# mederrata/spmf

Measured on AMD Instinct MI355X. Metric: elbo_steps_per_sec, higher is better.
Workload: dtype f32

## Files before the change

spmf_amd/csrc/row_pass.hip:

```cpp
#include <algorithm>

#include "common.h"
#include "kernels.h"

namespace spmf {

#ifndef ROW_MAX_BLOCKS
#define ROW_MAX_BLOCKS 4096
#endif
#ifndef ROW_DYN_NUM
#define ROW_DYN_NUM 1
#define ROW_DYN_DEN 8
#endif
static_assert(ROW_MAX_BLOCKS <= spmf::kDetMaxBlocks,
              "the deterministic mode's per-workgroup slots (common.h kDetMaxBlocks) are sized for at most that many row-pass workgroups");
#ifndef ROW_GRP
#define ROW_GRP 4
#endif
#ifndef ROW_WAVES_PER_SIMD
#define ROW_WAVES_PER_SIMD 1
#endif

namespace {

__device__ __forceinline__ float* lds_dyn() {
  extern __shared__ __attribute__((aligned(16))) float spmf_row_lds[];
  return spmf_row_lds;
}

template <int FMT>
struct EntryRow {
  __amdgpu_buffer_rsrc_t a, b;
};
template <int FMT>
__device__ __forceinline__ EntryRow<FMT> entry_row(const int32_t* __restrict__ col, const float* __restrict__ val,
                                                   const uint32_t* __restrict__ ent, int start, int n) {
  EntryRow<FMT> r;
  start = __builtin_amdgcn_readfirstlane(start);
  n = __builtin_amdgcn_readfirstlane(n);
  if (FMT == 1) {
    r.a = __builtin_amdgcn_make_buffer_rsrc(const_cast<uint32_t*>(ent + start), 0, n * 4, 0x00020000);
    r.b = r.a;
  } else {
    r.a = __builtin_amdgcn_make_buffer_rsrc(const_cast<int32_t*>(col + start), 0, n * 4, 0x00020000);
    r.b = __builtin_amdgcn_make_buffer_rsrc(const_cast<float*>(val + start), 0, n * 4, 0x00020000);
  }
  return r;
}
template <int FMT, bool NT>
__device__ __forceinline__ void load_entry(const EntryRow<FMT>& r, int i, int& ra, float& rb) {
  constexpr int AUX = NT ? 2 : 0;
  ra = (int)__builtin_amdgcn_raw_buffer_load_b32(r.a, i * 4, 0, AUX);
  rb = FMT == 1 ? 0.f : __uint_as_float(__builtin_amdgcn_raw_buffer_load_b32(r.b, i * 4, 0, AUX));
}
template <int FMT>
__device__ __forceinline__ void unpack_entry(int ra, float rb, bool ok, int& c, float& x) {
  if (FMT == 1) {
    const uint32_t w = ok ? (uint32_t)ra : kPadWord;
    c = (int)(w >> 16);
    x = (float)(w & 0xffffu);
  } else {
    c = ok ? ra : kPadRow;
    x = ok ? rb : 0.f;
  }
}

template <bool BASE>
__device__ __forceinline__ int bperm_i(int base_bytes, int imm_lanes, int v) {
  if constexpr (BASE) return __builtin_amdgcn_ds_bpermute(base_bytes + imm_lanes * 4, v);
  else return __shfl(v, (base_bytes >> 2) + imm_lanes);
}
template <bool BASE>
__device__ __forceinline__ float bperm_f(int base_bytes, int imm_lanes, float v) {
  return __int_as_float(bperm_i<BASE>(base_bytes, imm_lanes, __float_as_int(v)));
}

template <int KP, int LIK, bool LDSPHI = false>
struct RowCtx {
  static constexpr int LPN = KP / 4;
  static constexpr int NPI = 64 / LPN;
  static constexpr int GRP = LPN < ROW_GRP ? LPN : ROW_GRP;
  static constexpr bool BPI = LPN <= 8 && LIK != 1;
  GTable Ap, Vp;
  const float* phi;
  const uint8_t* ctype;
  int lane, sub, grp;
  int bp_grp, bp_row;

  template <int CNT>
  __device__ __forceinline__ void s1_group(int c, float x, int g0, float4& zacc) const {
    float4 a[CNT];
    float xv[CNT];
#pragma unroll
    for (int j = 0; j < CNT; ++j) {
      const int d = bperm_i<BPI>(bp_grp, (g0 + j) * NPI, c);
      xv[j] = bperm_f<BPI>(bp_grp, (g0 + j) * NPI, x);
      a[j] = gather4<LPN>(Ap, d, sub);
    }
#pragma unroll
    for (int j = 0; j < CNT; ++j) zacc = fma4(xv[j], a[j], zacc);
  }
  __device__ __forceinline__ void sweep1(int c, float x, int nchunk, float4& zacc) const {
#pragma unroll
    for (int g0 = 0; g0 < LPN; g0 += GRP) {
      if (g0 * NPI < nchunk) s1_group<GRP>(c, x, g0, zacc);
    }
  }

  template <int CNT>
  __device__ __forceinline__ void s2_issue(int c, int g0, float4 (&vv)[LPN]) const {
#pragma unroll
    for (int j = 0; j < CNT; ++j) {
      const int d = bperm_i<BPI>(bp_grp, (g0 + j) * NPI, c);
      vv[g0 + j] = gather4<LPN>(Vp, d, sub);
    }
  }
  template <int CNT>
  __device__ __forceinline__ void s2_dots(int g0, const float4& z, float4 (&vv)[LPN], float& rmine) const {
#pragma unroll
    for (int j = 0; j < CNT; ++j) {
      const float dot = group_sum<LPN>(dot4(z, vv[g0 + j]));
      if (sub == g0 + j) rmine = dot;
    }
#pragma unroll
    for (int j = CNT; j < GRP; ++j) vv[g0 + j] = make_float4(0.f, 0.f, 0.f, 0.f);
  }
  template <int CNT>
  __device__ __forceinline__ void s2_back(float cc, int g0, const float4 (&vv)[LPN],
                                          float4& gz) const {
#pragma unroll
    for (int j = 0; j < CNT; ++j) {
      const float cb = bperm_f<BPI>(bp_row, g0 + j, cc);
      gz = fma4(cb, vv[g0 + j], gz);
    }
  }

  __device__ __forceinline__ void s2_load(int c, int nchunk, float4 (&vv)[LPN]) const {
#pragma unroll
    for (int g0 = 0; g0 < LPN; g0 += GRP) {
      if (g0 * NPI < nchunk) {
#pragma unroll
        for (int j = 0; j < GRP; ++j) {
          const int d = bperm_i<BPI>(bp_grp, (g0 + j) * NPI, c);
          vv[g0 + j] = gather4<LPN>(Vp, d, sub);
        }
      } else {
#pragma unroll
        for (int j = 0; j < GRP; ++j) vv[g0 + j] = make_float4(0.f, 0.f, 0.f, 0.f);
      }
    }
  }
  __device__ __forceinline__ void sweep2_loaded(int c, float x, int nchunk, const float4& z, float4& gz, float& ll,
                                                double& nnf, const float4 (&vv)[LPN]) const {
    float rmine = 0.f;
#pragma unroll
    for (int g0 = 0; g0 < LPN; g0 += GRP) {
      if (g0 * NPI < nchunk) {
#pragma unroll
        for (int j = 0; j < GRP; ++j) {
          const float dot = group_sum<LPN>(dot4(z, vv[g0 + j]));
          if (sub == g0 + j) rmine = dot;
        }
      }
    }
    s2_cells(c, x, nchunk, rmine, vv, gz, ll, nnf);
  }

  template <class Hook>
  __device__ __forceinline__ void sweep2(int c, float x, int nchunk, const float4& z, float4& gz, float& ll,
                                         double& nnf, Hook&& behind_last) const {
    float4 vv[LPN];
    float rmine = 0.f;
#pragma unroll
    for (int g0 = 0; g0 < LPN; g0 += GRP) {
      const bool occ = g0 * NPI < nchunk;
      if (occ) s2_issue<GRP>(c, g0, vv);
      if (g0 + GRP >= LPN) behind_last();
      if (occ) s2_dots<GRP>(g0, z, vv, rmine);
      else s2_dots<0>(g0, z, vv, rmine);
    }
    s2_cells(c, x, nchunk, rmine, vv, gz, ll, nnf);
  }
  __device__ __forceinline__ void s2_cells(int c, float x, int nchunk, float rmine, const float4 (&vv)[LPN],
                                           float4& gz, float& ll, double& nnf) const {
    const int slot = sub * NPI + grp;
    const float xs = __shfl(x, slot);
    const int cs = __shfl(c, slot);
    float cc = 0.f;
    if (slot < nchunk && xs > 0.f) {
      if (LIK == 2 || LIK == 4 || (LIK == 3 && ctype[cs])) {
        float ey = 1.f;
        const float fy = LIK == 4 ? expm1_dec(fminf(rmine, kYSat), ey) : rmine;
        const float lg = fy + (LDSPHI ? lds_dyn()[cs] : phi[cs]);
        if (lg > -INFINITY && lg < INFINITY) {
          ll = fmaf(xs, lg, ll);
          cc = LIK == 4 ? xs * ey : xs;
        } else {
          nnf += 1.0;
        }
      } else {
        float ey = 1.f;
        const float fy = LIK == 1 ? expm1_dec(fminf(rmine, kYSat), ey) : rmine;
        const float r = fy + (LDSPHI ? lds_dyn()[cs] : phi[cs]);
        if (r > 0.f && r < INFINITY) {
          ll = fmaf(xs, logf(r), ll);
          cc = xs * ey * __builtin_amdgcn_rcpf(r);
        } else {
          nnf += 1.0;
          cc = ey;
        }
      }
    }
#pragma unroll
    for (int g0 = 0; g0 < LPN; g0 += GRP) {
      if (g0 * NPI < nchunk) s2_back<GRP>(cc, g0, vv, gz);
    }
  }
};

}

template <int KP, int LIK, int BT = 256, int PACKED = 0>
__global__ __launch_bounds__(BT, BT == 256 ? ROW_WAVES_PER_SIMD : 4) void row_pass_kernel(
    int64_t B, const int32_t* __restrict__ row_ptr, const int32_t* __restrict__ col,
    const float* __restrict__ val, const float* __restrict__ row_scale,
    const float* __restrict__ Ap, const float* __restrict__ Vp, const float* __restrict__ phi,
    const double* __restrict__ dprep, float* __restrict__ z, float* __restrict__ gzs,
    double* __restrict__ dacc, int mode, const float* __restrict__ gzd,
    const uint8_t* __restrict__ ctype, int Dcols, int64_t dacc_stride,
    const uint32_t* __restrict__ ent, double* __restrict__ det_slots, int64_t det_stride, int dyn_tail) {
  if (gridDim.y > 1) {
    const size_t sd = blockIdx.y;
    Ap += sd * (size_t)Dcols * KP;
    Vp += sd * (size_t)Dcols * KP;
    phi += sd * (size_t)Dcols;
    dprep += sd * (size_t)kPrepSeg * (KP + 1);
    z += sd * (size_t)B * KP;
    gzs += sd * (size_t)B * KP;
    dacc += sd * (size_t)dacc_stride;
  }
  const bool encode_only = mode == 1;
  constexpr int LPN = KP / 4;
  constexpr bool LDSPHI = BT != 256;
  if (LDSPHI && !encode_only) {
    float* pl = lds_dyn();
    for (int i = threadIdx.x; i < Dcols; i += BT) pl[i] = phi[i];
    __syncthreads();
  }
  RowCtx<KP, LIK, LDSPHI> cx;
  cx.Ap = gtable(Ap, Dcols, KP);
  cx.Vp = gtable(Vp, Dcols, KP);
  cx.phi = phi;
  cx.ctype = ctype;
  cx.lane = threadIdx.x & 63;
  cx.sub = cx.lane % LPN;
  cx.grp = cx.lane / LPN;
  cx.bp_grp = cx.grp * 4;
  cx.bp_row = cx.grp * LPN * 4;
  const int lane = cx.lane, sub = cx.sub, grp = cx.grp;
  const int wave = (int)blockIdx.x * (BT / 64) + __builtin_amdgcn_readfirstlane((int)(threadIdx.x >> 6));
  const int nwaves = (int)gridDim.x * (BT / 64);
  const int Bn = (int)B;

  float4 veta4 = make_float4(0.f, 0.f, 0.f, 0.f);
  if (!encode_only && (mode != 2 || LIK == 3 || !gzd))
    veta4 = make_float4((float)prep_sum(dprep, KP, sub * 4 + 0), (float)prep_sum(dprep, KP, sub * 4 + 1),
                        (float)prep_sum(dprep, KP, sub * 4 + 2), (float)prep_sum(dprep, KP, sub * 4 + 3));
  double ll_acc = 0.0, zsq_acc = 0.0, nnf_acc = 0.0;
  float4 zsum = make_float4(0.f, 0.f, 0.f, 0.f);

  int B_static = Bn;
  int dyn_lo = Bn, dyn_hi = Bn;
  unsigned int* dyn_ctr = nullptr;
  if (dyn_tail && !det_slots && !encode_only) {
    const int per_wave = Bn / nwaves;
    if (per_wave >= 8) {
      int fixed = per_wave - (per_wave * ROW_DYN_NUM) / ROW_DYN_DEN;
      if (fixed < 2) fixed = 2;
      B_static = fixed * nwaves;
      const int r = (int)(wave & (kDaccRep - 1));
      const int each = (Bn - B_static + kDaccRep - 1) / kDaccRep;
      dyn_lo = B_static + r * each;
      dyn_hi = dyn_lo + each < Bn ? dyn_lo + each : Bn;
      if (dyn_lo > Bn) dyn_lo = Bn;
      dyn_ctr = reinterpret_cast<unsigned int*>(dacc + (size_t)r * (kDaccHead + KP) + kDaccDynSlot);
    }
  }
  auto fixed_next = [&](int cur) -> int {
    if (cur >= Bn) return Bn;
    if (cur + nwaves < B_static) return cur + nwaves;
    return dyn_ctr ? -1 : Bn;
  };
  auto take_dynamic = [&]() -> int {
    unsigned int k = 0;
    if (lane == 0) k = atomicAdd(dyn_ctr, 1u);
    k = (unsigned int)__builtin_amdgcn_readfirstlane((int)k);
    const int row = dyn_lo + (int)k;
    return row < dyn_hi ? row : Bn;
  };

  const __amdgpu_buffer_rsrc_t dyn_rsrc = __builtin_amdgcn_make_buffer_rsrc(
      dyn_ctr ? dyn_ctr : reinterpret_cast<unsigned int*>(dacc), 0, dyn_ctr ? 4 : 0, 0x00020000);

  typedef const __attribute__((address_space(4))) int32_t* RowPtr;
  typedef const __attribute__((address_space(4))) float* RowScale;
  const RowPtr rptr = (RowPtr)row_ptr;
  const RowScale rscale = (RowScale)row_scale;
  int start = 0, end = 0, pc0 = 0, pc1 = 0, nstart = 0, nend = 0;
  float xi = 1.f, px0 = 0.f, px1 = 0.f, nxi = 1.f;
  int b = wave < B_static ? wave : Bn;
  int bn = fixed_next(b);
  if (bn < 0) bn = take_dynamic();
  int bnn = fixed_next(bn);
  if (bnn < 0) bnn = take_dynamic();
  if (b < Bn) {
    start = rptr[b];
    end = rptr[b + 1];
    xi = row_scale ? rscale[b] : 1.f;
    const EntryRow<PACKED> er = entry_row<PACKED>(col, val, ent, start, end - start);
    load_entry<PACKED, true>(er, lane, pc0, px0);
    load_entry<PACKED, true>(er, lane + 64, pc1, px1);
  }
  if (bn < Bn) {
    nstart = rptr[bn];
    nend = rptr[bn + 1];
    nxi = row_scale ? rscale[bn] : 1.f;
  }
  while (b < Bn) {
    const int n = end - start;
    int qc0 = 0, qc1 = 0, nnstart = 0, nnend = 0;
    float qx0 = 0.f, qx1 = 0.f, nnxi = 1.f;
    int bnnn = fixed_next(bnn);
    const bool dyn_ask = bnnn < 0;
    unsigned int dyn_k = 0;
    auto issue_next = [&]() {
      issue_fence(PACKED ? (const void*)ent : (const void*)col, val, row_ptr);
      dyn_k = (unsigned int)__builtin_amdgcn_raw_ptr_buffer_atomic_add_i32(1, dyn_rsrc, (dyn_ask && lane == 0) ? 0 : 4,
                                                                       0, 0);
      const EntryRow<PACKED> er = entry_row<PACKED>(col, val, ent, nstart, nend - nstart);
      load_entry<PACKED, true>(er, lane, qc0, qx0);
      load_entry<PACKED, true>(er, lane + 64, qc1, qx1);
      if (bnn < Bn) {
        nnstart = rptr[bnn];
        nnend = rptr[bnn + 1];
        nnxi = row_scale ? rscale[bnn] : 1.f;
      }
      issue_fence(PACKED ? (const void*)ent : (const void*)col, val, row_ptr);
    };
    constexpr bool BEHIND = KP <= 32;
    if constexpr (!BEHIND) issue_next();
    float4 zacc = make_float4(0.f, 0.f, 0.f, 0.f);
    float4 gz = make_float4(0.f, 0.f, 0.f, 0.f);
    float llrow = 0.f;
    if (n <= 128) {
      int c0, c1;
      float x0, x1;
      unpack_entry<PACKED>(pc0, px0, lane < n, c0, x0);
      unpack_entry<PACKED>(pc1, px1, lane + 64 < n, c1, x1);
      int n0 = min(n, 64);
      const int n1 = n - 64;
      if (mode != 2) {
        cx.sweep1(c0, x0, n0, zacc);
        if (n1 > 0) cx.sweep1(c1, x1, n1, zacc);
        zacc = across_groups_sum4<LPN>(zacc);
        zacc.x *= xi; zacc.y *= xi; zacc.z *= xi; zacc.w *= xi;
        if (grp == 0) reinterpret_cast<float4*>(z)[(size_t)b * LPN + sub] = zacc;
      } else {
        zacc = gather4<LPN>(z, (int)b, sub);
      }
      if (encode_only) {
        if constexpr (BEHIND) issue_next();
      } else {
        if constexpr (KP <= 32) {
          float4 vv[LPN];
          if (n1 > 0) {
            cx.s2_load(c0, n0, vv);
            cx.sweep2_loaded(c0, x0, n0, zacc, gz, llrow, nnf_acc, vv);
            c0 = c1; x0 = x1; n0 = n1;
          }
          cx.s2_load(c0, n0, vv);
          issue_next();
          cx.sweep2_loaded(c0, x0, n0, zacc, gz, llrow, nnf_acc, vv);
        } else {
          cx.sweep2(c0, x0, n0, zacc, gz, llrow, nnf_acc, [] {});
          if (n1 > 0) cx.sweep2(c1, x1, n1, zacc, gz, llrow, nnf_acc, [] {});
        }
      }
    } else {
      const EntryRow<PACKED> er = entry_row<PACKED>(col, val, ent, start, n);
      if (mode != 2) {
        int ra = pc0, ra1 = pc1;
        float rb = px0, rb1 = px1;
        for (int base = start; base < end; base += 64) {
          const int i2 = base + 128 + lane;
          int ra2;
          float rb2;
          load_entry<PACKED, false>(er, i2 - start, ra2, rb2);
          int c;
          float x;
          unpack_entry<PACKED>(ra, rb, base + lane < end, c, x);
          cx.sweep1(c, x, min(64, end - base), zacc);
          ra = ra1; rb = rb1; ra1 = ra2; rb1 = rb2;
        }
        zacc = across_groups_sum4<LPN>(zacc);
        zacc.x *= xi; zacc.y *= xi; zacc.z *= xi; zacc.w *= xi;
        if (grp == 0) reinterpret_cast<float4*>(z)[(size_t)b * LPN + sub] = zacc;
      } else {
        zacc = gather4<LPN>(z, (int)b, sub);
      }
      if (encode_only) {
        if constexpr (BEHIND) issue_next();
      } else {
        int ra = pc0, ra1 = pc1;
        float rb = px0, rb1 = px1;
        for (int base = start; base < end; base += 64) {
          const int i2 = base + 128 + lane;
          int ra2;
          float rb2;
          load_entry<PACKED, false>(er, i2 - start, ra2, rb2);
          int c;
          float x;
          unpack_entry<PACKED>(ra, rb, base + lane < end, c, x);
          if (BEHIND && base + 64 >= end) cx.sweep2(c, x, end - base, zacc, gz, llrow, nnf_acc, issue_next);
          else cx.sweep2(c, x, min(64, end - base), zacc, gz, llrow, nnf_acc, [] {});
          ra = ra1; rb = rb1; ra1 = ra2; rb1 = rb2;
        }
      }
    }
    const float xi_cur = xi;
    const int b_cur = b;
    start = nstart; end = nend; xi = nxi;
    pc0 = qc0; px0 = qx0; pc1 = qc1; px1 = qx1;
    nstart = nnstart; nend = nnend; nxi = nnxi;
    {
      const int row = dyn_lo + (int)(unsigned int)__builtin_amdgcn_readfirstlane((int)dyn_k);
      if (dyn_ask) bnnn = row < dyn_hi ? row : Bn;
    }
    b = bn; bn = bnn; bnn = bnnn;
    if (encode_only) continue;
    gz = across_groups_sum4<LPN>(gz);
    if (grp == 0) {
      zsq_acc += (double)dot4(zacc, zacc);
      zsum = add4(zsum, zacc);
      float4 dn = (mode == 2 && gzd) ? gather4<LPN>(gzd, (int)b_cur, sub) : veta4;
      if (LIK == 3 && mode == 2 && gzd) dn = add4(dn, veta4);
      if (mode == 3 && LIK != 3) dn = make_float4(0.f, 0.f, 0.f, 0.f);
      float4 o;
      o.x = xi_cur * (gz.x - dn.x - zacc.x);
      o.y = xi_cur * (gz.y - dn.y - zacc.y);
      o.z = xi_cur * (gz.z - dn.z - zacc.z);
      o.w = xi_cur * (gz.w - dn.w - zacc.w);
      reinterpret_cast<float4*>(gzs)[(size_t)b_cur * LPN + sub] = o;
    }
    ll_acc += (double)llrow;
  }
  if (encode_only) return;

  __shared__ double red[16];
  __shared__ double zred_static[BT == 256 ? 4 : 1][KP];
  if (LDSPHI) __syncthreads();
  double (*zred)[KP] = LDSPHI ? reinterpret_cast<double (*)[KP]>(lds_dyn()) : zred_static;
  const int wid = threadIdx.x >> 6;
  if (grp == 0) {
    zred[wid][sub * 4 + 0] = (double)zsum.x;
    zred[wid][sub * 4 + 1] = (double)zsum.y;
    zred[wid][sub * 4 + 2] = (double)zsum.z;
    zred[wid][sub * 4 + 3] = (double)zsum.w;
  }
  const double ll_b = block_sum(ll_acc, red);
  const double zq_b = block_sum(zsq_acc, red);
  const double nf_b = block_sum(nnf_acc, red);
  if (det_slots) {
    double* sl = det_slots + (size_t)blockIdx.y * det_stride;
    if (blockIdx.x == 0 && threadIdx.x == 0) sl[0] = (double)gridDim.x;
    sl += kDetMeta + (size_t)blockIdx.x * (kDaccHead + KP);
    if (threadIdx.x == 0) {
      sl[0] = ll_b;
      sl[1] = zq_b;
      sl[2] = nf_b;
      sl[3] = sl[4] = sl[5] = 0.0;
    }
    __syncthreads();
    if (threadIdx.x < KP) {
      double t = 0.0;
      const int nw = blockDim.x >> 6;
      for (int i = 0; i < nw; ++i) t += zred[i][threadIdx.x];
      sl[kDaccHead + threadIdx.x] = t;
    }
    return;
  }
  dacc += (size_t)(blockIdx.x % kDaccRep) * (kDaccHead + KP);
  if (threadIdx.x == 0) {
    atomicAdd(&dacc[0], ll_b);
    atomicAdd(&dacc[1], zq_b);
    if (nf_b != 0.0) atomicAdd(&dacc[2], nf_b);
  }
  __syncthreads();
  if (threadIdx.x < KP) {
    double t = 0.0;
    const int nw = blockDim.x >> 6;
    for (int i = 0; i < nw; ++i) t += zred[i][threadIdx.x];
    atomicAdd(&dacc[kDaccHead + threadIdx.x], t);
  }
}

template <int KP, int LIK, int BT, int PACKED>
static bool launch_row_lds_t(const RowArgs& a, hipStream_t st) {
  const size_t lds = a.mode == 1 ? 0 : std::max((size_t)a.D * 4, (size_t)(BT / 64) * KP * sizeof(double));
  constexpr int kMaxDev = 64;
  static size_t granted[kMaxDev] = {};
  if (lds > 64 * 1024) {
    int dev = 0;
    if (hipGetDevice(&dev) != hipSuccess || dev < 0 || dev >= kMaxDev) {
      (void)hipGetLastError();
      return false;
    }
    if (lds > __atomic_load_n(&granted[dev], __ATOMIC_RELAXED)) {
      if (hipFuncSetAttribute((const void*)row_pass_kernel<KP, LIK, BT, PACKED>,
                              hipFuncAttributeMaxDynamicSharedMemorySize, (int)lds) != hipSuccess) {
        (void)hipGetLastError();
        return false;
      }
      __atomic_store_n(&granted[dev], lds, __ATOMIC_RELAXED);
    }
  }
  const int64_t want = (a.B + (BT / 64) - 1) / (BT / 64);
#ifndef ROW_LDS_CAP
#define ROW_LDS_CAP 1024
#endif
  const int64_t cap = (int64_t)ROW_LDS_CAP * 256 / BT;
  const int nb = (int)(want < 1 ? 1 : (want > cap ? cap : want));
  hipLaunchKernelGGL((row_pass_kernel<KP, LIK, BT, PACKED>), dim3(nb, a.S > 1 ? a.S : 1), dim3(BT), lds, st,
                     a.B, a.row_ptr, a.col, a.val, a.row_scale, a.Ap, a.Vp, a.phi, a.dprep, a.z,
                     a.gzs, a.dacc, a.mode, a.gzd, a.ctype, a.D, a.dacc_stride, a.ent, a.det_slots, a.det_stride, a.dyn_tail);
  return true;
}

template <int KP, int LIK, int BT>
static bool launch_row_lds(const RowArgs& a, hipStream_t st) {
  return a.ent ? launch_row_lds_t<KP, LIK, BT, 1>(a, st) : launch_row_lds_t<KP, LIK, BT, 0>(a, st);
}

template <int KP>
static bool launch_row_t(const RowArgs& a, hipStream_t st) {
  int64_t want = (a.B + 3) / 4;
  int nb = (int)(want < 1 ? 1 : (want > ROW_MAX_BLOCKS ? ROW_MAX_BLOCKS : want));
  if constexpr (KP >= 16) {
    if (a.mode == 1 && a.B >= 4096) {
      if (launch_row_lds<KP, 0, 512>(a, st)) return true;
    }
    if (a.mode != 1 && a.logt >= 0 && a.logt <= 3 && a.B >= 4096) {
      const size_t need = (size_t)a.D * 4;
      bool done = false;
      if (need <= 80 * 1024) {
        done = a.logt == 0   ? launch_row_lds<KP, 0, 512>(a, st)
               : a.logt == 1 ? launch_row_lds<KP, 1, 512>(a, st)
               : a.logt == 2 ? launch_row_lds<KP, 2, 512>(a, st)
                             : launch_row_lds<KP, 3, 512>(a, st);
      } else if (need <= 160 * 1024 - 1024) {
        done = a.logt == 0   ? launch_row_lds<KP, 0, 1024>(a, st)
               : a.logt == 1 ? launch_row_lds<KP, 1, 1024>(a, st)
               : a.logt == 2 ? launch_row_lds<KP, 2, 1024>(a, st)
                             : launch_row_lds<KP, 3, 1024>(a, st);
      }
      if (done) return true;
    }
  }
#define SPMF_ROW_LAUNCH(L_)                                                                    \
  hipLaunchKernelGGL((row_pass_kernel<KP, L_>), dim3(nb, a.S > 1 ? a.S : 1), dim3(256), 0, st, \
                     a.B, a.row_ptr, a.col, a.val, a.row_scale, a.Ap, a.Vp, a.phi, a.dprep, a.z, \
                     a.gzs, a.dacc, a.mode, a.gzd, a.ctype, a.D, a.dacc_stride, a.ent, a.det_slots, a.det_stride, a.dyn_tail)
  if (a.logt == 4) SPMF_ROW_LAUNCH(4);
  else if (a.logt == 3) SPMF_ROW_LAUNCH(3);
  else if (a.logt == 2) SPMF_ROW_LAUNCH(2);
  else if (a.logt == 1) SPMF_ROW_LAUNCH(1);
  else SPMF_ROW_LAUNCH(0);
#undef SPMF_ROW_LAUNCH
  return true;
}

bool launch_row_pass(int KP, const RowArgs& a, hipStream_t st) {
  if (KP > 64) return launch_row_widek(KP, a, st);
  bool ok = false;
  return with_kp<64>(KP, [&](auto kp) { ok = launch_row_t<decltype(kp)::value>(a, st); }) && ok;
}

}
```

Baseline: 386.6.

## Specialize short-row sweeps by exact gather count via compile-time switch arms

For KP<=32, the last chunk of a short row is dispatched through a switch to an arm templated on the exact number of occupied gather slots. Encode and decode sweeps then issue only the needed gathers, dots and back-projections instead of group-granular predicated loops. The launch bounds for KP==32 are also changed to allow more waves per SIMD, which caps register use. In exchange, code size grows with up to eight unrolled arms, and the tighter register cap may cause spills.

```diff
diff --git a/spmf_amd/csrc/row_pass.hip b/spmf_amd/csrc/row_pass.hip
--- a/spmf_amd/csrc/row_pass.hip
+++ b/spmf_amd/csrc/row_pass.hip
@@ -135,35 +135,57 @@
     }
   }
 
-  __device__ __forceinline__ void s2_load(int c, int nchunk, float4 (&vv)[LPN]) const {
-#pragma unroll
-    for (int g0 = 0; g0 < LPN; g0 += GRP) {
-      if (g0 * NPI < nchunk) {
-#pragma unroll
-        for (int j = 0; j < GRP; ++j) {
-          const int d = bperm_i<BPI>(bp_grp, (g0 + j) * NPI, c);
-          vv[g0 + j] = gather4<LPN>(Vp, d, sub);
-        }
-      } else {
-#pragma unroll
-        for (int j = 0; j < GRP; ++j) vv[g0 + j] = make_float4(0.f, 0.f, 0.f, 0.f);
-      }
-    }
-  }
-  __device__ __forceinline__ void sweep2_loaded(int c, float x, int nchunk, const float4& z, float4& gz, float& ll,
-                                                double& nnf, const float4 (&vv)[LPN]) const {
+
+  template <int T>
+  __device__ __forceinline__ void s1_arm(int c, float x, float4& zacc) const {
+    constexpr int WHOLE = T / GRP * GRP;
+#pragma unroll
+    for (int g0 = 0; g0 < WHOLE; g0 += GRP) s1_group<GRP>(c, x, g0, zacc);
+    if constexpr (T > WHOLE) s1_group<T - WHOLE>(c, x, WHOLE, zacc);
+  }
+  template <int T, class Hook>
+  __device__ __forceinline__ void s2_arm(int c, float x, int nchunk, const float4& z, float4& gz, float& ll,
+                                         double& nnf, Hook&& behind) const {
+    float4 vv[LPN];
     float rmine = 0.f;
-#pragma unroll
-    for (int g0 = 0; g0 < LPN; g0 += GRP) {
-      if (g0 * NPI < nchunk) {
-#pragma unroll
-        for (int j = 0; j < GRP; ++j) {
-          const float dot = group_sum<LPN>(dot4(z, vv[g0 + j]));
-          if (sub == g0 + j) rmine = dot;
-        }
-      }
-    }
-    s2_cells(c, x, nchunk, rmine, vv, gz, ll, nnf);
+    s2_issue<T>(c, 0, vv);
+    behind();
+    if constexpr (T > 0) {
+#pragma unroll
+      for (int j = 0; j < T; ++j) {
+        const float dot = group_sum<LPN>(dot4(z, vv[j]));
+        if (sub == j) rmine = dot;
+      }
+      s2_cells<T>(c, x, nchunk, rmine, vv, gz, ll, nnf);
+    }
+  }
+  template <class F>
+  __device__ __forceinline__ static void by_count(int t, F&& f) {
+    static_assert(LPN <= 8, "the arms are written out up to eight gather instructions per chunk");
+#define SPMF_ROW_ARM(T_)                                            \
+  case T_:                                                          \
+    if constexpr (LPN >= T_) f(std::integral_constant<int, T_>{});  \
+    break;
+    switch (t) {
+      SPMF_ROW_ARM(1) SPMF_ROW_ARM(2) SPMF_ROW_ARM(3) SPMF_ROW_ARM(4)
+      SPMF_ROW_ARM(5) SPMF_ROW_ARM(6) SPMF_ROW_ARM(7) SPMF_ROW_ARM(8)
+      default: f(std::integral_constant<int, 0>{}); break;
+    }
+#undef SPMF_ROW_ARM
+  }
+  __device__ __forceinline__ static int count_of(int n) { return (int)((unsigned)(n + NPI - 1) / (unsigned)NPI); }
+  __device__ __forceinline__ void sweep1_last(int c, float x, int nlast, float4& zacc) const {
+    by_count(count_of(nlast), [&](auto t) __attribute__((always_inline)) {
+      constexpr int T = decltype(t)::value;
+      if constexpr (T > 0) s1_arm<T>(c, x, zacc);
+    });
+  }
+  template <class Hook>
+  __device__ __forceinline__ void sweep2_last(int c, float x, int nlast, const float4& z, float4& gz, float& ll,
+                                              double& nnf, Hook&& behind) const {
+    by_count(count_of(nlast), [&](auto t) __attribute__((always_inline)) {
+      s2_arm<decltype(t)::value>(c, x, nlast, z, gz, ll, nnf, behind);
+    });
   }
 
   template <class Hook>
@@ -181,6 +203,7 @@
     }
     s2_cells(c, x, nchunk, rmine, vv, gz, ll, nnf);
   }
+  template <int CNT = -1>
   __device__ __forceinline__ void s2_cells(int c, float x, int nchunk, float rmine, const float4 (&vv)[LPN],
                                            float4& gz, float& ll, double& nnf) const {
     const int slot = sub * NPI + grp;
@@ -211,9 +234,13 @@
         }
       }
     }
-#pragma unroll
-    for (int g0 = 0; g0 < LPN; g0 += GRP) {
-      if (g0 * NPI < nchunk) s2_back<GRP>(cc, g0, vv, gz);
+    if constexpr (CNT >= 0) {
+      s2_back<CNT>(cc, 0, vv, gz);
+    } else {
+#pragma unroll
+      for (int g0 = 0; g0 < LPN; g0 += GRP) {
+        if (g0 * NPI < nchunk) s2_back<GRP>(cc, g0, vv, gz);
+      }
     }
   }
 };
@@ -221,7 +248,7 @@
 }
 
 template <int KP, int LIK, int BT = 256, int PACKED = 0>
-__global__ __launch_bounds__(BT, BT == 256 ? ROW_WAVES_PER_SIMD : 4) void row_pass_kernel(
+__global__ __launch_bounds__(BT, BT == 256 && KP != 32 ? ROW_WAVES_PER_SIMD : 4) void row_pass_kernel(
     int64_t B, const int32_t* __restrict__ row_ptr, const int32_t* __restrict__ col,
     const float* __restrict__ val, const float* __restrict__ row_scale,
     const float* __restrict__ Ap, const float* __restrict__ Vp, const float* __restrict__ phi,
@@ -333,7 +360,7 @@
     int bnnn = fixed_next(bnn);
     const bool dyn_ask = bnnn < 0;
     unsigned int dyn_k = 0;
-    auto issue_next = [&]() {
+    auto issue_next = [&]() __attribute__((always_inline)) {
       issue_fence(PACKED ? (const void*)ent : (const void*)col, val, row_ptr);
       dyn_k = (unsigned int)__builtin_amdgcn_raw_ptr_buffer_atomic_add_i32(1, dyn_rsrc, (dyn_ask && lane == 0) ? 0 : 4,
                                                                        0, 0);
@@ -357,11 +384,19 @@
       float x0, x1;
       unpack_entry<PACKED>(pc0, px0, lane < n, c0, x0);
       unpack_entry<PACKED>(pc1, px1, lane + 64 < n, c1, x1);
-      int n0 = min(n, 64);
+      const int n0 = min(n, 64);
       const int n1 = n - 64;
+      const bool two = n1 > 0;
+      const int cl = two ? c1 : c0, nl = two ? n1 : n0;
+      const float xl = two ? x1 : x0;
       if (mode != 2) {
-        cx.sweep1(c0, x0, n0, zacc);
-        if (n1 > 0) cx.sweep1(c1, x1, n1, zacc);
+        if constexpr (KP <= 32) {
+          if (two) cx.template s1_arm<LPN>(c0, x0, zacc);
+          cx.sweep1_last(cl, xl, nl, zacc);
+        } else {
+          cx.sweep1(c0, x0, n0, zacc);
+          if (two) cx.sweep1(c1, x1, n1, zacc);
+        }
         zacc = across_groups_sum4<LPN>(zacc);
         zacc.x *= xi; zacc.y *= xi; zacc.z *= xi; zacc.w *= xi;
         if (grp == 0) reinterpret_cast<float4*>(z)[(size_t)b * LPN + sub] = zacc;
@@ -372,15 +407,8 @@
         if constexpr (BEHIND) issue_next();
       } else {
         if constexpr (KP <= 32) {
-          float4 vv[LPN];
-          if (n1 > 0) {
-            cx.s2_load(c0, n0, vv);
-            cx.sweep2_loaded(c0, x0, n0, zacc, gz, llrow, nnf_acc, vv);
-            c0 = c1; x0 = x1; n0 = n1;
-          }
-          cx.s2_load(c0, n0, vv);
-          issue_next();
-          cx.sweep2_loaded(c0, x0, n0, zacc, gz, llrow, nnf_acc, vv);
+          if (two) cx.template s2_arm<LPN>(c0, x0, 64, zacc, gz, llrow, nnf_acc, [] {});
+          cx.sweep2_last(cl, xl, nl, zacc, gz, llrow, nnf_acc, issue_next);
         } else {
           cx.sweep2(c0, x0, n0, zacc, gz, llrow, nnf_acc, [] {});
           if (n1 > 0) cx.sweep2(c1, x1, n1, zacc, gz, llrow, nnf_acc, [] {});
```

After: 393.9 (median of 6 runs). +1.9%, better.
